# fractalclockwork/CS267_HW3

Hardware: NVIDIA B200
Metric: kmers_per_s_insert_plus_traverse (higher is better)
Workload: dtype u128

## Files before the change

### cs267_hw3_b200/csrc/capi.cu

```cuda
#include <algorithm>
#include <cmath>
#include <cstdio>
#include <cstdlib>
#include <cstring>
#include <string>
#include <vector>

#include <cub/device/device_radix_sort.cuh>

#include "../../include/kh_capi.h"
#include "kernels.cuh"
#include "ctable.cuh"

using namespace kh;

namespace {

struct DevBuf {
    void* p = nullptr;
    size_t cap = 0;
};

enum { EV_INS0, EV_INS1, EV_AS0, EV_WALK, EV_RANK, EV_AS1, EV_PACK0, EV_PACK1, EV_CLR0, EV_CLR1, EV_STAGE1, EV_BUILD0, EV_BUILD1, EV_COUNT };

// ... 672 lines not shown
template <int W>
int ct_assemble_part(kh_table* t, int part) {
    typedef typename Slot<W>::value_t V;
    auto& c = t->ct;
    const unsigned gb = (unsigned)t->sm_count * 8;
    u64* link = static_cast<u64*>(t->link.p);
    CtGathered gt = {};
    for (int r = 0; r < c.pe.world; ++r) {
        const bool me = r == c.pe.rank;
        gt.link[r] = me ? link : static_cast<const u64*>(c.g_link.p) + (u64)r * c.caps.g_seg_stride;
        gt.meta[r] = me ? static_cast<const u64*>(c.meta.p) : static_cast<const u64*>(c.g_meta.p) + (u64)r * c.caps.g_seg_stride;
        gt.pool[r] = me ? static_cast<const unsigned char*>(c.pool.p) : static_cast<const unsigned char*>(c.g_pool.p) + (u64)r * c.caps.g_pool_stride;
    }
    switch (part) {
    case 0:
        if (c.assembled) { c.sealed = false; c.assembled = false; }
        c.slow = false;
        KH_CUDA(t, cudaEventRecord(t->ev[EV_AS0], t->stream));
        if (!c.sealed) return ct_seal_publish<W>(t);
        return ct_barrier(t);
    case 1: {
        if (!c.sealed) { KH_TRY(ct_seal_build<W>(t)); KH_CUDA(t, cudaEventRecord(t->ev[EV_INS1], t->stream)); t->have_ins = true; }
        if (!c.sharded) {
            const u64 hc = c.n_starts_host;
            KH_TRY(ensure(t, t->contig_len, (hc + 3) * sizeof(u32)));
            KH_TRY(ensure(t, t->contig_pre, (hc + 3) * sizeof(u32)));
            KH_TRY(ensure(t, t->contig_off, (hc + 3) * sizeof(u64)));
            c.out_cap = t->h_ctr->n_inserted + c.n_starts_host * (u64)(t->k + 1) + 64;
            ct_set_self(t);
        }
        if (c.pe.world > 1) {
            KH_CUDA(t, cudaEventRecord(t->ev_built, t->stream));
            KH_CUDA(t, cudaStreamWaitEvent(t->copy_stream, t->ev_built, 0));
            ct_gather_kernel<<<gb, 256, 0, t->copy_stream>>>(c.pe, c.caps, link, static_cast<const u64*>(c.meta.p), static_cast<const unsigned char*>(c.pool.p),
                                                             static_cast<const u32*>(c.pool_off.p), c.g.chunks_per_rank, t->d_ctr, 0);
            KH_CUDA(t, cudaEventRecord(t->ev_gathered, t->copy_stream));
            ++t->n_launches;
        }
        ct_init_assemble_kernel<<<1, 1, 0, t->stream>>>(t->d_ctr);
        KH_CUDA(t, cudaMemsetAsync(c.out_cursor.p, 0, kMaxRanks * sizeof(u32), t->stream));
        ct_stub_kernel<W><<<std::max(1u, std::min(gb, (c.caps.hcap + 255u) / 256u)), 256, 0, t->stream>>>(
            static_cast<const V*>(t->starts.p), t->d_ctr, c.caps.hcap, link, static_cast<u64*>(c.meta.p), static_cast<V*>(c.ext_key.p));
        ct_resolve_kernel<W><<<gb, 256, 0, t->stream>>>(static_cast<const V*>(t->table), static_cast<const u32*>(c.chunk_base.p),
                                                        static_cast<const u32*>(c.seg_base.p), link, static_cast<const V*>(c.ext_key.p),
                                                        c.g, c.pe, c.caps, static_cast<u32*>(c.out_cursor.p), static_cast<u32*>(c.req_seg.p), t->d_ctr);
        if (c.pe.world > 1) { ct_publish_inbox_kernel<<<1, 32, 0, t->stream>>>(c.pe, c.caps, static_cast<const u32*>(c.out_cursor.p)); ++t->n_launches; }
        t->n_launches += 3;
        KH_CUDA(t, cudaGetLastError());
        return ct_barrier(t);
    }
    case 2:
        if (c.pe.world > 1) {
            ct_answer_kernel<W><<<gb, 256, 0, t->stream>>>(static_cast<const V*>(t->table), static_cast<const u32*>(c.chunk_base.p),
                                                           static_cast<const u32*>(c.seg_base.p), static_cast<const CtReq<W>*>(c.inbox.p),
                                                           static_cast<const u32*>(c.inbox_cnt.p), c.g, c.pe, c.caps);
            KH_CUDA(t, cudaGetLastError());
            ++t->n_launches;
        }
        return ct_barrier(t);
    case 3:
        if (c.pe.world > 1) {
            ct_apply_kernel<<<gb, 256, 0, t->stream>>>(link, static_cast<const u32*>(c.answers.p), static_cast<const u32*>(c.req_seg.p),
                                                       static_cast<const u32*>(c.out_cursor.p), c.caps, c.pe.world, c.pe.rank);
            ct_gather_kernel<<<gb, 256, 0, t->stream>>>(c.pe, c.caps, link, static_cast<const u64*>(c.meta.p), static_cast<const unsigned char*>(c.pool.p),
                                                        static_cast<const u32*>(c.pool_off.p), c.g.chunks_per_rank, t->d_ctr, 1);
            KH_CUDA(t, cudaStreamWaitEvent(t->stream, t->ev_gathered, 0));
            KH_CUDA(t, cudaGetLastError());
            t->n_launches += 2;
        }
        KH_CUDA(t, cudaEventRecord(t->ev[EV_WALK], t->stream));
        return ct_barrier(t);
    case 4:
        ct_walk_len_kernel<<<gb, 256, 0, t->stream>>>(gt, link, c.caps, t->k, kCtWalkMaxSteps, static_cast<u32*>(t->contig_len.p), t->d_ctr);
        KH_CUDA(t, cudaGetLastError());
        ++t->n_launches;
        return ct_barrier(t, -2);
    case 5: {
        KH_TRY(device_scan(t, static_cast<u32*>(t->contig_len.p), (u64)c.caps.hcap + 1, static_cast<u64*>(t->contig_off.p), &t->d_ctr->contig_bytes));
        KH_CUDA(t, cudaEventRecord(t->ev[EV_RANK], t->stream));
        ct_walk_emit_kernel<W><<<gb, 256, 0, t->stream>>>(gt, link, static_cast<const V*>(t->starts.p), c.caps, t->k, static_cast<const u32*>(t->contig_len.p),
                                                          static_cast<const u64*>(t->contig_off.p), c.out_cap, static_cast<char*>(t->out.p), t->d_ctr);
        KH_CUDA(t, cudaGetLastError());
        ++t->n_launches;
        KH_CUDA(t, cudaEventRecord(t->ev[EV_AS1], t->stream));
        t->have_as = true;
        return KH_OK;
    }
    case 6: {
        KH_TRY(read_counters(t));
        c.slow = (c.pe.world > 1 ? t->h_ctr->use_jump : t->h_ctr->need_jump) != 0;
        if (!c.slow) return KH_OK;
        c.assembled = true;
        ct_rank_round_kernel<<<gb, 256, 0, t->stream>>>(c.pe, link, c.caps, t->d_ctr, t->d_ctr->flags, 0);
        KH_CUDA(t, cudaGetLastError());
        ++t->n_launches;
        return ct_barrier(t, 0);
    }
    case 6 + kCtMaxRounds: {
        if (!c.slow) return KH_OK;
        ct_reset_nodes_kernel<<<1, 1, 0, t->stream>>>(t->d_ctr);
        ct_lengths_kernel<<<gb, 256, 0, t->stream>>>(c.pe, link, c.caps, t->k, static_cast<u32*>(t->contig_len.p),
                                                     static_cast<u32*>(t->contig_pre.p), t->d_ctr);
        ct_claim_kernel<<<gb, 256, 0, t->stream>>>(c.pe, link, c.caps, static_cast<const u32*>(t->contig_len.p), t->d_ctr);
        KH_CUDA(t, cudaGetLastError());
        t->n_launches += 3;
        KH_TRY(device_scan(t, static_cast<u32*>(t->contig_len.p), (u64)c.caps.hcap + 1, static_cast<u64*>(t->contig_off.p), &t->d_ctr->contig_bytes));
        KH_CUDA(t, cudaEventRecord(t->ev[EV_RANK], t->stream));
        return ct_barrier(t);
    }
    case 7 + kCtMaxRounds:
        if (!c.slow) return KH_OK;
        ct_emit_kernel<<<gb, 256, 0, t->stream>>>(c.pe, link, static_cast<const u64*>(c.meta.p), static_cast<const unsigned char*>(c.pool.p),
                                                  c.caps, t->d_ctr, t->k);
        ct_emit_heads_kernel<W><<<gb, 256, 0, t->stream>>>(static_cast<const V*>(t->starts.p), c.caps, t->k, static_cast<const u32*>(t->contig_len.p),
                                                          static_cast<const u64*>(t->contig_off.p), t->d_ctr, c.out_cap, static_cast<char*>(t->out.p));
        KH_CUDA(t, cudaGetLastError());
        t->n_launches += 2;
        KH_CUDA(t, cudaEventRecord(t->ev[EV_AS1], t->stream));
        t->have_as = true;
        return ct_barrier(t);
    default: {
        if (part < 7 || part >= 6 + kCtMaxRounds) return fail(t, KH_ERR_ARG, "unknown assemble part");
        if (!c.slow) return KH_OK;
        const int r = part - 6;
        ct_rank_round_kernel<<<gb, 256, 0, t->stream>>>(c.pe, link, c.caps, t->d_ctr, t->d_ctr->flags, r);
        KH_CUDA(t, cudaGetLastError());
        ++t->n_launches;
        return ct_barrier(t, r);
    }
    }
}

int ct_finish(kh_table* t, u32* bits_out) {
    auto& c = t->ct;
    KH_TRY(read_counters(t));
    const Counters& h = *t->h_ctr;
    const u64 n_starts = std::min<u64>(h.n_starts_dev, c.caps.hcap);
    t->n_starts = n_starts;
    t->stats.n_contigs = n_starts;
    t->stats.n_nodes = h.n_nodes;
    t->stats.contig_bytes = h.contig_bytes;
    t->stats.n_segments = (h.next_seg > c.caps.hcap ? h.next_seg - c.caps.hcap : 0) + n_starts;
    u32 rounds = 0;
    for (int i = 0; i < kCtMaxRounds; ++i) rounds += h.flags[i] ? 1u : 0u;
    t->stats.rank_rounds = rounds + 1;
    t->last_contig_bytes = h.contig_bytes;
    t->last_n_contigs = n_starts;
    u32 e = h.errors;
    if (e == 0 && h.contig_bytes > c.out_cap) e = kErrConverge;
    if (bits_out) *bits_out = e;
    if (e & kErrInternal) {
        char msg[512];
        snprintf(msg, sizeof msg, "rank %d/%d internal error, site bits 0x%x (1 barrier wait, 2 start list, 4 segment ids, 8 link inbox, "
                 "16 unresolved head stub, 32 output buffer): starts %llu/%u, segments %u/%u, contig bytes %llu/%llu, epoch %u",
                 c.pe.rank, c.pe.world, h.err_where, (unsigned long long)h.n_starts_dev, c.caps.hcap, h.next_seg, c.caps.seg_cap,
                 (unsigned long long)h.contig_bytes, (unsigned long long)c.out_cap, c.epoch);
        t->err = msg;
        fprintf(stderr, "libkh_b200: %s\n", msg);
    }
    if (h.errors) { clear_error_bits(t); KH_CUDA(t, cudaMemsetAsync(&t->d_ctr->err_where, 0, sizeof(u32), t->stream)); }
    return KH_OK;
}

template <int W>
int ct_insert_plain(kh_table* t, const unsigned char* recs, u64 n, bool record_start) {
    auto& c = t->ct;
    if (record_start) KH_CUDA(t, cudaEventRecord(t->ev[EV_INS0], t->stream));
    KH_TRY(ct_stage<W>(t, recs, n));
    KH_TRY(read_counters(t));
    c.n_starts_host = std::min<u64>(t->h_ctr->n_starts_dev, 0xFFFFFF00ull);
    t->n_starts = c.n_starts_host;
    KH_CUDA(t, cudaEventRecord(t->ev[EV_INS1], t->stream));
    t->have_ins = true;
    const u32 e = t->h_ctr->errors;
    if (e) { clear_error_bits(t); return status_from_errors(t, e); }
    return KH_OK;
}

template <int W>
int ct_seal_plain(kh_table* t) {
    auto& c = t->ct;
    if (c.sealed) return KH_OK;
    KH_TRY(ct_seal_publish<W>(t));
    KH_TRY(ct_seal_build<W>(t));
    KH_CUDA(t, cudaEventRecord(t->ev[EV_INS1], t->stream));
    KH_TRY(read_counters(t));
    const u32 e = t->h_ctr->errors;
    if (e) { clear_error_bits(t); return status_from_errors(t, e); }
    return KH_OK;
}

template <int W>
int ct_assemble_plain(kh_table* t) {
    auto& c = t->ct;
    if (c.assembled) { c.sealed = false; c.assembled = false; }
    KH_TRY(ct_seal_plain<W>(t));
    KH_TRY(ensure(t, t->out, t->h_ctr->n_inserted + c.n_starts_host * (u64)(t->k + 1) + 64));
    for (int part = 0; part < kCtParts; ++part) KH_TRY(ct_assemble_part<W>(t, part));
    u32 bits = 0;
    KH_TRY(ct_finish(t, &bits));
    if (bits) return status_from_errors(t, bits);
    return KH_OK;
}

}

extern "C" {

int kh_abi_version(void) { return 2; }

int kh_device_count(void) {
    int n = 0;
    if (cudaGetDeviceCount(&n) != cudaSuccess) { cudaGetLastError(); return 0; }
    return n;
}

const char* kh_status_string(int s) {
    switch (s) {
    case KH_OK: return "ok";
    case KH_ERR_ARG: return "bad argument";
    case KH_ERR_CUDA: return "CUDA failure or no CUDA device";
    case KH_ERR_NOT_FOUND: return "Error: k-mer not found in Distributed HashMap.";
    case KH_ERR_TABLE_FULL: return "hash table full";
    case KH_ERR_CYCLE: return "chain never terminates (cycle)";
    case KH_ERR_BAD_INPUT: return "malformed input";
    case KH_ERR_CONVERGE: return "chains are not linear (shared end node)";
    case KH_ERR_NOMEM: return "out of memory";
    default: return "unknown status";
    }
}

uint64_t kh_packed_bytes(int k) { return (uint64_t)((k + 3) / 4); }
uint64_t kh_pair_bytes(int k) { return (uint64_t)((k + 3) / 4 + 2); }

int kh_create(int k, uint64_t n_expected, double load_factor, int device, kh_table** out) {
    if (!out) return KH_ERR_ARG;
    *out = nullptr;
    if (k < 2 || k > 61 || !(load_factor > 0.0) || load_factor > 1.0) return KH_ERR_ARG;
    int ndev = 0;
    if (cudaGetDeviceCount(&ndev) != cudaSuccess || ndev == 0) { cudaGetLastError(); return KH_ERR_CUDA; }
    if (device < 0 || device >= ndev) return KH_ERR_ARG;
    kh_table* t = new kh_table();
    auto bail = [&](int rc) { kh_destroy(t); return rc; };
    t->k = k; t->device = device; t->lf = load_factor; t->n_expected = n_expected;
    t->pl = (k + 3) / 4; t->pb = t->pl + 2;
    t->ct_env = env_int("KH_CT", 1);
    const bool use_ct = ct_supported(k) && (t->ct_env == 2 || (t->ct_env != 0 && n_expected >= (1ull << 20) && 2 * k + 6 > 64));
    t->W = use_ct ? ct_slot_words(k) : ((2 * k + 6 <= 64) ? 1 : 2);
    t->slot_bytes = t->W == 1 ? 8 : 16;
    t->per_bucket = 32 / t->slot_bytes;
    if (cudaSetDevice(device) != cudaSuccess) return bail(KH_ERR_CUDA);
    cudaDeviceProp prop;
    if (cudaGetDeviceProperties(&prop, device) != cudaSuccess) return bail(KH_ERR_CUDA);
    if (prop.major < 9) { fprintf(stderr, "libkh_b200: device %d is sm_%d%d; this library is built for sm_100a only\n", device, prop.major, prop.minor); return bail(KH_ERR_CUDA); }
    t->sm_count = prop.multiProcessorCount;
    const int gran = env_int("KH_L2_FETCH_BYTES", 32);
    if (gran > 0) { cudaDeviceSetLimit(cudaLimitMaxL2FetchGranularity, (size_t)gran); cudaGetLastError(); }

    const long double slots = (long double)std::max<uint64_t>(n_expected, 1) / (long double)load_factor;
    t->nbuckets = std::max<u64>(16, (u64)(slots / t->per_bucket) + 1);
    t->nbuckets = (t->nbuckets + 15) / 16 * 16;
    t->table_bytes = use_ct ? 0 : (size_t)t->nbuckets * 32;
    int rc = KH_OK;
    auto ck = [&](cudaError_t e) { if (e != cudaSuccess && rc == KH_OK) { rc = e == cudaErrorMemoryAllocation ? KH_ERR_NOMEM : KH_ERR_CUDA; t->err = cudaGetErrorString(e); } };
    ck(cudaStreamCreateWithFlags(&t->own_stream, cudaStreamNonBlocking));
    ck(cudaStreamCreateWithFlags(&t->copy_stream, cudaStreamNonBlocking));
    t->stream = t->own_stream;
    if (!use_ct) ck(cudaMalloc(&t->table, t->table_bytes));
    ck(cudaMalloc((void**)&t->d_ctr, sizeof(Counters)));
    ck(cudaHostAlloc((void**)&t->h_ctr, sizeof(Counters), cudaHostAllocDefault));
    for (auto& e : t->ev) ck(cudaEventCreate(&e));
    for (auto& e : t->ev_copied) ck(cudaEventCreateWithFlags(&e, cudaEventDisableTiming));
    for (auto& e : t->ev_consumed) ck(cudaEventCreateWithFlags(&e, cudaEventDisableTiming));
    ck(cudaEventCreateWithFlags(&t->ev_built, cudaEventDisableTiming));
    ck(cudaEventCreateWithFlags(&t->ev_gathered, cudaEventDisableTiming));
    if (rc != KH_OK) { fprintf(stderr, "libkh_b200: kh_create: %s\n", t->err.c_str()); return bail(rc); }
    if (!use_ct) ck(cudaMemsetAsync(t->table, 0, t->table_bytes, t->stream));
    ck(cudaMemsetAsync(t->d_ctr, 0, sizeof(Counters), t->stream));
    ck(cudaStreamSynchronize(t->stream));
    if (rc != KH_OK) return bail(rc);
    memset(t->h_ctr, 0, sizeof(Counters));
    int v = env_int("KH_SPLIT_BUCKETS", 0);
    if (v > 0 && set_option(t, "split_buckets", v) != KH_OK) fprintf(stderr, "libkh_b200: ignoring KH_SPLIT_BUCKETS=%d\n", v);
    t->partition_mode = env_int("KH_PARTITION", -1);
    t->build_mode = env_int("KH_BUILD", t->W == 1 ? 1 : 0);
    t->debug_cap_pct = std::max(1, env_int("KH_DEBUG_CAP_PCT", 100));
    v = env_int("KH_SEG_CHARS", 0);
    if (v > 0 && set_option(t, "seg_chars", v) != KH_OK) fprintf(stderr, "libkh_b200: ignoring KH_SEG_CHARS=%d\n", v);
    if (use_ct) {
        rc = t->W == 1 ? ct_setup<1>(t, 0, 1, n_expected, n_expected, n_expected, false)
                       : ct_setup<2>(t, 0, 1, n_expected, n_expected, n_expected, false);
        if (rc != KH_OK) { fprintf(stderr, "libkh_b200: kh_create: %s\n", t->err.c_str()); return bail(rc); }
    }
    t->err.clear();
    *out = t;
    return KH_OK;
}

int kh_destroy(kh_table* t) {
    if (!t) return KH_OK;
    cudaSetDevice(t->device);
    if (t->own_stream) cudaStreamSynchronize(t->own_stream);
    DevBuf* bufs[] = {&t->starts, &t->mask, &t->tile_counts, &t->tile_offs, &t->scan_blocks, &t->link, &t->seglen,
                      &t->tmp, &t->part_cursor, &t->grouped, &t->fine, &t->chunk_cursor, &t->overflow, &t->contig_len, &t->contig_pre, &t->contig_off, &t->out, &t->stage[0], &t->stage[1],
                      &t->text_stage, &t->scratch_a, &t->scratch_b, &t->scratch_c, &t->sort_keys[0], &t->sort_keys[1], &t->sort_vals[0], &t->sort_vals[1], &t->sort_tmp};
    for (DevBuf* b : bufs) if (b->p) cudaFree(b->p);
    for (auto& row : t->ct.ipc_opened) for (void* q : row) if (q) cudaIpcCloseMemHandle(q);
// ... 596 lines not shown
```

### cs267_hw3_b200/csrc/ctable.cuh

```cuda
#pragma once
#include "kernels.cuh"

namespace kh {

#ifndef KH_CT_BUCKETS2
#define KH_CT_BUCKETS2 2176
#endif
#ifndef KH_CT_THREADS
#define KH_CT_THREADS 512
#endif
#ifndef KH_CT_MINBLOCKS
#define KH_CT_MINBLOCKS 2
#endif
#ifndef KH_CT_JUMPS
#define KH_CT_JUMPS 3
#endif
template <int W> struct CtBuild {
    static constexpr u32 kMaxBuckets = (W == 1) ? 1536u : (u32)KH_CT_BUCKETS2;
    static constexpr u32 kMaxSlots = kMaxBuckets * (u32)Slot<W>::kPerBucket;
    static constexpr u32 kOffSucc = kMaxBuckets * 32u;
    static constexpr u32 kOffPd = kOffSucc + kMaxSlots * 2u;
    static constexpr u32 kOffOff = kOffPd + kMaxSlots * 4u;
    static constexpr u32 kOffCode = kOffOff + kMaxSlots * 2u;
    static constexpr u32 kSmem = kOffCode + kMaxSlots;
};
constexpr int kCtBuildThreads = KH_CT_THREADS;
template <int W>
__host__ __device__ __forceinline__ u64 ct_fine_index(u32 chunk, u32 at, u32 nchunks) {
    constexpr u32 G = 128u / (u32)sizeof(typename Slot<W>::value_t);
    return ((u64)(at / G) * nchunks + chunk) * G + (at % G);
}
constexpr u32 kSuccExt = 0x8000u, kSuccTail = 0xFFFFu, kSuccDead = 0xFFFDu, kPredNone = 0xFFFFu;
constexpr u32 kCodeBackF = 8u, kCodeMulti = 16u;

template <int W> struct CtReq;
template <> struct alignas(16) CtReq<1> { u64 key; u32 src; u32 chunk; };
template <> struct alignas(16) CtReq<2> { u128 key; u32 src; u32 chunk; u64 pad; };

struct CtPeers {
    int world, rank;
    void* xin_vals[kMaxRanks];
    u32* xin_chunk[kMaxRanks];
    u32* xin_cnt[kMaxRanks];
    void* extra_vals[kMaxRanks];
    u32* extra_chunk[kMaxRanks];
    u32* extra_cnt[kMaxRanks];
    u64* link[kMaxRanks];
    u64* meta[kMaxRanks];
    void* inbox[kMaxRanks];
    u32* inbox_cnt[kMaxRanks];
    u32* answers[kMaxRanks];
    u64* g_link[kMaxRanks];
    u64* g_meta[kMaxRanks];
    unsigned char* g_pool[kMaxRanks];
    u32* g_hdr[kMaxRanks];
    u32* contig_pre[kMaxRanks];
    u64* contig_off[kMaxRanks];
    char* out[kMaxRanks];
    u64 out_cap[kMaxRanks];
    u32* flags[kMaxRanks];
};

struct CtCaps {
    u32 xin_cap, extra_cap, inbox_cap, seg_cap, hcap;
    u64 nbuckets_alloc, pool_cap;
    u64 g_seg_stride, g_pool_stride;
};

__device__ __forceinline__ void ct_internal(Counters* ctr, u32 site) {
    atomicOr(&ctr->errors, kErrInternal);
    atomicOr(&ctr->err_where, site);
}

__global__ void ct_barrier_kernel(const CtPeers pe, u32 epoch, Counters* ctr, int round) {
    const int r = (int)threadIdx.x;
    if (round >= 0 && ctr->rank_done) return;
    const u32 bit = round >= 0 ? (ctr->flags[round] ? 1u : 0u) : (round == -2 ? (ctr->need_jump ? 1u : 0u) : 0u);
    u32 peer_bit = 0;
    if (r < pe.world) {
        __threadfence_system();
        u32* dst = pe.flags[r] + 2 * pe.rank + (epoch & 1u);
        asm volatile("st.release.sys.global.u32 [%0], %1;" ::"l"(dst), "r"((epoch << 1) | bit) : "memory");
        const u32* src = pe.flags[pe.rank] + 2 * r + (epoch & 1u);
        unsigned long long t0, t1;
        asm volatile("mov.u64 %0, %%globaltimer;" : "=l"(t0));
        for (;;) {
            u32 seen;
            asm volatile("ld.acquire.sys.global.u32 %0, [%1];" : "=r"(seen) : "l"(src) : "memory");
            if ((int)((seen >> 1) - epoch) >= 0) { peer_bit = ((seen >> 1) == epoch) ? (seen & 1u) : (round >= 0 ? 0u : 1u); break; }
            asm volatile("mov.u64 %0, %%globaltimer;" : "=l"(t1));
            if (t1 - t0 > 4000000000ull) { ct_internal(ctr, kSiteBarrier); peer_bit = 1; break; }
            __nanosleep(200);
        }
        __threadfence_system();
    }
    if (round >= 0) {
        const u32 any = __ballot_sync(kFullMask, peer_bit != 0);
        if (r == 0 && any == 0) ctr->rank_done = 1;
    } else if (round == -2) {
        const u32 any = __ballot_sync(kFullMask, peer_bit != 0);
        if (r == 0) ctr->use_jump = any ? 1u : 0u;
    }
}

template <int W> __device__ __forceinline__ typename Slot<W>::value_t ct_record_from_words(const u32 (&w)[W == 1 ? 3 : 5], u32 sh, int k, int pl, bool& ok);
template <> __device__ __forceinline__ u64 ct_record_from_words<1>(const u32 (&w)[3], u32 sh, int k, int pl, bool& ok) {
    const u32 b0 = __funnelshift_r(w[0], w[1], sh), b1 = __funnelshift_r(w[1], w[2], sh);
    const u64 be = ((u64)__byte_perm(b0, 0, 0x0123) << 32) | (u64)__byte_perm(b1, 0, 0x0123);
    const u64 key = be >> (64 - 2 * k);
    const u32 ext = (u32)((((u64)b1 << 32) | b0) >> (8 * pl));
    const u32 b = ext_code((unsigned char)ext), f = ext_code((unsigned char)(ext >> 8));
    ok = (b != kExtBad) && (f != kExtBad);
    return (key << 6) | ((u64)(b & 7u) << 3) | (u64)((f + 1u) & 7u);
}
template <> __device__ __forceinline__ u128 ct_record_from_words<2>(const u32 (&w)[5], u32 sh, int k, int pl, bool& ok) {
    const u32 b0 = __funnelshift_r(w[0], w[1], sh), b1 = __funnelshift_r(w[1], w[2], sh);
    const u32 b2 = __funnelshift_r(w[2], w[3], sh), b3 = __funnelshift_r(w[3], w[4], sh);
    const u64 hi = ((u64)__byte_perm(b0, 0, 0x0123) << 32) | (u64)__byte_perm(b1, 0, 0x0123);
    const u64 lo = ((u64)__byte_perm(b2, 0, 0x0123) << 32) | (u64)__byte_perm(b3, 0, 0x0123);
    u128 v = Slot<2>::shr_any(u128{lo, hi}, 122 - 2 * k);
    const int wq = pl >> 2;
    const u32 e0 = wq == 1 ? b1 : (wq == 2 ? b2 : b3), e1 = wq == 1 ? b2 : (wq == 2 ? b3 : 0u);
    const u32 ext = __funnelshift_r(e0, e1, 8u * (pl & 3));
    const u32 b = ext_code((unsigned char)ext), f = ext_code((unsigned char)(ext >> 8));
    ok = (b != kExtBad) && (f != kExtBad);
    v.lo = (v.lo & ~63ull) | ((u64)(b & 7u) << 3) | (u64)((f + 1u) & 7u);
    return v;
}

constexpr int kStgThreads = 256;
constexpr int kStgPer = 4;
constexpr int kStgTile = kStgThreads * kStgPer;

template <int W>
__global__ void __launch_bounds__(kStgThreads, 5)
ct_stage_kernel(const unsigned char* __restrict__ recs, u64 n, const CtGeom g, const CtPeers pe, const CtCaps caps,
                u32* __restrict__ chunk_cursor, typename Slot<W>::value_t* __restrict__ fine, u32* __restrict__ xout_cursor,
                u32* __restrict__ start_mask, u32* __restrict__ tile_starts, Counters* ctr) {
    typedef Slot<W> S;
    typedef typename S::value_t V;
    constexpr u32 kMaxSlots = CtBuild<W>::kMaxSlots;
    extern __shared__ __align__(16) unsigned char s_raw[];
    V* s_sorted = reinterpret_cast<V*>(s_raw);
    u32* s_schunk = reinterpret_cast<u32*>(s_raw + (size_t)kStgTile * sizeof(V));
    __shared__ u32 s_cnt[kMaxRanks], s_off[kMaxRanks + 1], s_gbase[kMaxRanks];
    __shared__ u32 s_starts[kStgTile / kInsTile], s_err;
    const int k = g.k, pl = (k + 3) >> 2, pb = pl + 2;
    const u64 rec0 = (u64)blockIdx.x * kStgTile;
    const u32 cnt = (u32)min((u64)kStgTile, n - rec0);
    const bool multi = g.world > 1;
    if (threadIdx.x < kMaxRanks) s_cnt[threadIdx.x] = 0;
    if (threadIdx.x < kStgTile / kInsTile) s_starts[threadIdx.x] = 0;
    if (threadIdx.x == 0) s_err = 0;
    constexpr int kWords = W == 1 ? 3 : 5;
    u32 raw[kStgPer][kWords];
    u32 shift[kStgPer];
#pragma unroll
    for (int r = 0; r < kStgPer; ++r) {
        const u32 j = threadIdx.x + r * kStgThreads;
        const u64 addr = reinterpret_cast<u64>(recs) + (rec0 + j) * (u64)pb;
        shift[r] = ((u32)addr & 3u) * 8u;
        const u32* wp = reinterpret_cast<const u32*>(addr & ~3ull);
        const u64 end = reinterpret_cast<u64>(recs) + n * (u64)pb;
#pragma unroll
        for (int q = 0; q < kWords; ++q)
            raw[r][q] = (j < cnt && reinterpret_cast<u64>(wp + q) < end) ? __ldg(wp + q) : 0u;
    }
    __syncthreads();
    V v[kStgPer];
    u32 dst[kStgPer];
    u32 at[kStgPer];
    u32 own[kStgPer];
    u32 err = 0;
#pragma unroll
    for (int r = 0; r < kStgPer; ++r) {
        const u32 j = threadIdx.x + r * kStgThreads;
        bool ok = true, live = j < cnt;
        dst[r] = 0xFFFFFFFFu; own[r] = 0xFFFFFFFFu; at[r] = 0;
        v[r] = ct_record_from_words<W>(raw[r], shift[r], k, pl, ok);
        if (!live) v[r] = S::zero();
        if (live && !ok) { err |= kErrBadInput; live = false; }
        if (live) {
            u32 owner, chunk;
            ct_place(ct_min_hash<W>(v[r], g.m, g.win), g, owner, chunk);
            dst[r] = chunk;
            if (!multi || owner == (u32)g.rank) at[r] = atomicAdd(&chunk_cursor[chunk], 1u);
// ... 255 lines not shown
        const bool m = (((q[i] ^ key) << kIdxBits) >> (kIdxBits + 6)) == 0ull;
        res = e ? kFindMiss : (m ? (int)(q[i] >> (64 - kIdxBits)) - 1 : res);
    }
    return res;
}
template <> __device__ __forceinline__ int ct_find_step<2>(unsigned saddr, u128 key) {
    u64 q[4];
    ct_lds_bucket<2>(saddr, q);
    int res = kFindNext;
#pragma unroll
    for (int i = 1; i >= 0; --i) {
        const bool e = ((u32)q[2 * i] & 7u) == 0u;
        const bool m = (((q[2 * i + 1] ^ key.hi) << kIdxBits) | ((q[2 * i] ^ key.lo) >> 6)) == 0ull;
        res = e ? kFindMiss : (m ? (int)(q[2 * i + 1] >> (64 - kIdxBits)) - 1 : res);
    }
    return res;
}

template <int W>
__global__ void __launch_bounds__(kCtBuildThreads, KH_CT_MINBLOCKS)
ct_build_kernel(const typename Slot<W>::value_t* __restrict__ fine, const u32* __restrict__ chunk_cursor,
                const u32* __restrict__ chunk_base, const u32* __restrict__ pool_off,
                typename Slot<W>::value_t* __restrict__ table, u32* __restrict__ seg_base,
                u64* __restrict__ link, u64* __restrict__ meta, typename Slot<W>::value_t* __restrict__ ext_key,
                unsigned char* __restrict__ pool, const CtGeom g, const CtCaps caps, Counters* ctr) {
    typedef Slot<W> S;
    typedef CtSlot<W> CS;
    typedef typename S::value_t V;
    typedef CtBuild<W> B;
    extern __shared__ __align__(128) unsigned char s_bld[];
    unsigned char* const s_raw = s_bld;
    V* s_tab = reinterpret_cast<V*>(s_raw);
    unsigned short* s_succ = reinterpret_cast<unsigned short*>(s_raw + B::kOffSucc);
    unsigned char* s_pool = s_raw + B::kOffSucc;
    u32* s_pd = reinterpret_cast<u32*>(s_raw + B::kOffPd);
    unsigned short* s_off = reinterpret_cast<unsigned short*>(s_raw + B::kOffOff);
    unsigned char* s_code = s_raw + B::kOffCode;
    __shared__ u32 s_inserted, s_dups, s_nheads, s_seg0, s_chars, s_err;
    const u32 c = blockIdx.x;
    const u32 b0 = chunk_base[c], nb = chunk_base[c + 1] - b0;
    const u32 cnt = min(chunk_cursor[c], B::kMaxSlots);
    if (nb == 0) {
        if (threadIdx.x == 0) seg_base[c] = 0;
        return;
    }
    const unsigned s_base = (unsigned)__cvta_generic_to_shared(s_tab);
    const int k = g.k;
    constexpr int kBatch = 4;
    V v[kBatch];
#pragma unroll
    for (int r = 0; r < kBatch; ++r) {
        const u32 i = threadIdx.x + r * kCtBuildThreads;
        v[r] = i < cnt ? fine[ct_fine_index<W>(c, i, g.chunks_per_rank)] : S::zero();
    }
    if (threadIdx.x == 0) { s_inserted = 0; s_dups = 0; s_nheads = 0; s_chars = 0; s_err = 0; }
    {
        uint4* s4 = reinterpret_cast<uint4*>(s_raw);
        for (u32 i = threadIdx.x; i < nb * 2u; i += kCtBuildThreads) s4[i] = make_uint4(0, 0, 0, 0);
        for (u32 i = threadIdx.x; i < cnt; i += kCtBuildThreads) s_pd[i] = (kPredNone << 16) | 1u;
    }
    __syncthreads();
    u32 inserted = 0, dups = 0, err = 0;
    for (u32 base = 0; base < cnt; base += kCtBuildThreads * kBatch) {
        V nxt[kBatch];
#pragma unroll
        for (int r = 0; r < kBatch; ++r) {
            const u32 i = base + kCtBuildThreads * kBatch + threadIdx.x + r * kCtBuildThreads;
            nxt[r] = i < cnt ? fine[ct_fine_index<W>(c, i, g.chunks_per_rank)] : S::zero();
        }
#pragma unroll
        for (int r = 0; r < kBatch; ++r) {
            const u32 node = base + threadIdx.x + r * kCtBuildThreads;
            if (node >= cnt) continue;
            const int slot = ct_smem_insert<W>(s_tab, s_base, nb, CS::with_idx(v[r], node + 1u));
            inserted += (slot >= 0);
            dups += (slot == -1);
            if (slot == -2) err |= kErrTableFull;
            s_succ[node] = (unsigned short)(slot >= 0 ? (u32)slot : kSuccDead);
        }
#pragma unroll
        for (int r = 0; r < kBatch; ++r) v[r] = nxt[r];
    }
    inserted = __reduce_add_sync(kFullMask, inserted);
    dups = __reduce_add_sync(kFullMask, dups);
    err = __reduce_or_sync(kFullMask, err);
    if (lane_id() == 0) {
        if (inserted) atomicAdd(&s_inserted, inserted);
        if (dups) atomicAdd(&s_dups, dups);
        if (err) atomicOr(&s_err, err);
    }
    __syncthreads();
#pragma unroll 1
    for (u32 base = threadIdx.x; base < cnt; base += 2 * kCtBuildThreads) {
        u32 slot[2], b[2], code[2];
        V key[2];
        int res[2];
#pragma unroll
        for (int q = 0; q < 2; ++q) {
            const u32 node = base + q * kCtBuildThreads;
            slot[q] = node < cnt ? (u32)s_succ[node] : kSuccDead;
        }
#pragma unroll
        for (int q = 0; q < 2; ++q) {
            const V cur = slot[q] != kSuccDead ? s_tab[slot[q]] : S::zero();
            const u32 f = slot[q] != kSuccDead ? S::fwd(cur) : kExtF;
            code[q] = f | ((slot[q] != kSuccDead && S::back(cur) == kExtF) ? kCodeBackF : 0u);
            key[q] = S::next_key(CS::strip(cur), k);
            b[q] = ct_bucket_in_chunk(CS::hash32(key[q]), nb);
        }
#pragma unroll
        for (int q = 0; q < 2; ++q) res[q] = (code[q] & 7u) != kExtF ? ct_find_step<W>(s_base + b[q] * 32u, key[q]) : kFindMiss;
#pragma unroll
        for (int q = 0; q < 2; ++q) {
            for (u32 tries = 1; res[q] == kFindNext && tries < nb; ++tries) {
                b[q] = (b[q] + 1 == nb) ? 0u : b[q] + 1;
                res[q] = ct_find_step<W>(s_base + b[q] * 32u, key[q]);
            }
        }
#pragma unroll
        for (int q = 0; q < 2; ++q) {
            const u32 node = base + q * kCtBuildThreads;
            if (node >= cnt) continue;
            s_code[node] = (unsigned char)code[q];
            u32 sc = slot[q] == kSuccDead ? kSuccDead : kSuccTail;
            if ((code[q] & 7u) != kExtF) {
                if (res[q] < 0) {
                    sc = kSuccExt | slot[q];
                } else {
                    sc = (u32)res[q];
                    s_pd[res[q]] = (node << 16) | 1u;
                }
            }
            s_succ[node] = (unsigned short)sc;
        }
    }
    __syncthreads();
#pragma unroll 1
    for (u32 node = threadIdx.x; node < cnt; node += kCtBuildThreads) {
        const u32 s = s_succ[node];
        if (s < kSuccExt && (s_pd[s] >> 16) != node) s_code[s] |= (unsigned char)kCodeMulti;
    }
    __syncthreads();
    for (u32 base = 0; base < cnt; base += kCtBuildThreads) {
        const u32 node = base + threadIdx.x;
        bool head = false, dead = true;
        if (node < cnt) {
            dead = s_succ[node] == kSuccDead;
            head = !dead && ((s_pd[node] >> 16) == kPredNone || (s_code[node] & (kCodeBackF | kCodeMulti)));
        }
        const u32 bal = __ballot_sync(kFullMask, head);
        u32 first = 0;
        if (lane_id() == 0 && bal) first = atomicAdd(&s_nheads, (u32)__popc(bal));
        first = __shfl_sync(kFullMask, first, 0);
        if (head) s_pd[node] = (node << 16) | (first + __popc(bal & ((1u << lane_id()) - 1u)));
        else if (dead && node < cnt) s_pd[node] = node << 16;
    }
    __syncthreads();
    const u32 nheads = s_nheads;
    if (threadIdx.x == 0) {
        u32 seg0 = nheads ? atomicAdd(&ctr->next_seg, nheads) : 0u;
        if (seg0 + nheads > caps.seg_cap) { ct_internal(ctr, kSiteSegCap); seg0 = caps.seg_cap; }
        s_seg0 = seg0;
        seg_base[c] = seg0;
    }
    u32 active = 0;
#pragma unroll 1
    for (u32 i = 0, node = threadIdx.x; node < cnt; ++i, node += kCtBuildThreads) {
        const u32 pd = s_pd[node];
        active |= ((pd >> 16) != node) ? (1u << i) : 0u;
    }
    for (int round = 0; round < (14 + KH_CT_JUMPS - 1) / KH_CT_JUMPS; ++round) {
#pragma unroll 1
        for (int rep = 0; rep < KH_CT_JUMPS; ++rep) {
#pragma unroll 1
            for (u32 m = active; m; m &= m - 1u) {
                const u32 i = (u32)__ffs((int)m) - 1u, node = threadIdx.x + i * kCtBuildThreads;
                const u32 pd = s_pd[node], a = pd >> 16;
                const u32 pa = s_pd[a], a2 = pa >> 16;
                if (a2 == a) { active &= ~(1u << i); continue; }
                s_pd[node] = (a2 << 16) | ((pd + pa) & 0xFFFFu);
            }
        }
        if (!__syncthreads_or(active != 0u)) break;
    }
    __syncthreads();
    const u32 seg0 = s_seg0;
    const u32 my_bits = (u32)g.rank << kRankShift;
    const u64 pool0 = pool_off[c];
    if (seg0 < caps.seg_cap) {
    #pragma unroll 1
    for (u32 node = threadIdx.x; node < cnt; node += kCtBuildThreads) {
            const u32 s = s_succ[node];
            if (s == kSuccDead) continue;
            const u32 pd = s_pd[node], a = pd >> 16;
            const bool root = a == node;
            const u32 pa = root ? pd : s_pd[a];
            if ((pa >> 16) != a) continue;
            const u32 f = s_code[node] & 7u;
            bool last = f == kExtF || s >= kSuccExt;
            u32 next_hi = f == kExtF ? kLinkTail : kLinkPending;
            if (!last) {
                const u32 ps = s_pd[s];
                if ((ps >> 16) == s) { last = true; next_hi = my_bits | (seg0 + (ps & 0xFFFFu)); }
            }
            if (!last) continue;
            const u32 n = (root ? 0u : (pd & 0xFFFFu)) + (f != kExtF ? 1u : 0u);
            const u32 off = atomicAdd(&s_chars, n);
            s_off[a] = (unsigned short)off;
            const u32 gseg = seg0 + (pa & 0xFFFFu);
            link[gseg] = ((u64)next_hi << 32) | (next_hi == kLinkTail ? 0u : n);
            meta[gseg] = ((pool0 + off) << 24) | n;
            if (next_hi == kLinkPending) ext_key[gseg] = S::next_key(CS::strip(s_tab[s & 0x7FFFu]), k);
        }
    }
    __syncthreads();
#pragma unroll 1
    for (u32 node = threadIdx.x; node < cnt; node += kCtBuildThreads) {
        const u32 code = s_code[node];
        if ((code & 7u) == kExtF) continue;
        const u32 pd = s_pd[node], a = pd >> 16;
        const bool root = a == node;
        if (!root && (s_pd[a] >> 16) != a) continue;
        s_pool[(u32)s_off[a] + (root ? 0u : (pd & 0xFFFFu))] = ext_char(code & 7u);
    }
    {
        const u32 nslots = nb * S::kPerBucket;
        for (u32 i = threadIdx.x; i < nslots; i += kCtBuildThreads) {
            const V cur = s_tab[i];
            if (S::empty(cur)) continue;
            const u32 node = CS::idx(cur) - 1u, pd = s_pd[node];
            s_tab[i] = CS::with_idx(cur, (pd >> 16) == node ? (pd & 0xFFFFu) + 1u : 0u);
        }
    }
    asm volatile("fence.proxy.async.shared::cta;" ::: "memory");
    __syncthreads();
    {
        const u32 tab_bytes = nb * 32u, pool_bytes = (s_chars + 15u) & ~15u;
        constexpr u32 kPiece = 8192u;
        const u32 tab_pieces = (tab_bytes + kPiece - 1u) / kPiece, pool_pieces = (pool_bytes + kPiece - 1u) / kPiece;
        if (lane_id() == 0) {
            unsigned char* g_tab = reinterpret_cast<unsigned char*>(table + (u64)b0 * S::kPerBucket);
            bool any = false;
            for (u32 pc = threadIdx.x >> 5; pc < tab_pieces + pool_pieces; pc += kCtBuildThreads / 32) {
                const bool is_tab = pc < tab_pieces;
                const u32 o = (is_tab ? pc : pc - tab_pieces) * kPiece;
                const u32 bytes = min(kPiece, (is_tab ? tab_bytes : pool_bytes) - o);
                const unsigned src = (unsigned)__cvta_generic_to_shared(is_tab ? s_raw + o : s_pool + o);
                unsigned char* dst = is_tab ? g_tab + o : pool + pool0 + o;
                asm volatile("cp.async.bulk.global.shared::cta.bulk_group [%0], [%1], %2;" ::"l"(dst), "r"(src), "r"(bytes) : "memory");
                any = true;
            }
            if (any) {
                asm volatile("cp.async.bulk.commit_group;" ::: "memory");
                asm volatile("cp.async.bulk.wait_group.read 0;" ::: "memory");
            }
        }
    }
    if (threadIdx.x == 0) {
        if (s_inserted) atomicAdd(&ctr->n_inserted, (u64)s_inserted);
        if (s_dups) atomicAdd(&ctr->n_duplicates, (u64)s_dups);
        if (s_err) atomicOr(&ctr->errors, s_err);
    }
}

template <int W>
__device__ __forceinline__ bool ct_lookup_chunk(const typename Slot<W>::value_t* __restrict__ table, const u32* __restrict__ chunk_base,
                                                u32 chunk, typename Slot<W>::value_t key, typename Slot<W>::value_t& found) {
    typedef Slot<W> S;
    typedef typename S::value_t V;
    const u32 b0 = chunk_base[chunk], nb = chunk_base[chunk + 1] - b0;
    if (nb == 0) return false;
    u32 b = ct_bucket_in_chunk(CtSlot<W>::hash32(key), nb);
    for (u32 tries = 0; tries < nb; ++tries) {
        u64 q[4];
        load256_nc(table + (u64)(b0 + b) * S::kPerBucket, q);
        bool hole = false, hit = false;
#pragma unroll
        for (int i = 0; i < S::kPerBucket; ++i) {
            const V cur = S::from_bucket(q, i);
            const bool e = S::empty(cur);
            if (!hole && !hit && !e && CtSlot<W>::same_key(cur, key)) { found = cur; hit = true; }
            hole = hole || e;
        }
        if (hit) return true;
        if (hole) return false;
        b = (b + 1 == nb) ? 0u : b + 1;
    }
    return false;
}

template <int W>
__global__ void __launch_bounds__(256)
ct_find_kernel(const typename Slot<W>::value_t* __restrict__ table, const u32* __restrict__ chunk_base, const CtGeom g,
               const unsigned char* __restrict__ pkmers, u64 n, unsigned char* __restrict__ pairs_out,
               unsigned char* __restrict__ found_out) {
    typedef Slot<W> S;
    const u64 i = (u64)blockIdx.x * blockDim.x + threadIdx.x;
    if (i >= n) return;
    const int k = g.k, pl = (k + 3) >> 2, pb = pl + 2;
    unsigned char key[16];
    for (int j = 0; j < pl; ++j) key[j] = pkmers[i * pl + j];
    const typename S::value_t kb = S::from_packed(key, k, pl);
    u32 owner, chunk;
    ct_place(ct_min_hash<W>(kb, g.m, g.win), g, owner, chunk);
    typename S::value_t hit;
    const bool ok = ct_lookup_chunk<W>(table, chunk_base, chunk, kb, hit);
    unsigned char rec[18];
    for (int j = 0; j < pb; ++j) rec[j] = 0;
    if (ok) S::to_record(CtSlot<W>::strip(hit), k, pl, rec);
    for (int j = 0; j < pb; ++j) pairs_out[i * pb + j] = rec[j];
    found_out[i] = ok ? 1 : 0;
}

template <int W>
__global__ void __launch_bounds__(256)
ct_stub_kernel(const typename Slot<W>::value_t* __restrict__ starts, const Counters* __restrict__ ctr, u32 hcap,
               u64* __restrict__ link, u64* __restrict__ meta, typename Slot<W>::value_t* __restrict__ ext_key) {
    typedef Slot<W> S;
    const u32 n_starts = (u32)min(ctr->n_starts_dev, (u64)hcap);
    for (u32 c = blockIdx.x * blockDim.x + threadIdx.x; c < hcap; c += gridDim.x * blockDim.x) {
        if (c < n_starts) {
            link[c] = (u64)kLinkPending << 32;
            meta[c] = 0;
            ext_key[c] = S::key_only(starts[c]);
        } else {
            link[c] = (u64)kLinkUnused << 32;
        }
    }
}

template <int W>
__device__ __forceinline__ u32 ct_resolve_one(const typename Slot<W>::value_t* __restrict__ table, const u32* __restrict__ chunk_base,
                                              const u32* __restrict__ seg_base, u32 chunk, typename Slot<W>::value_t key, u32 my_bits) {
    typename Slot<W>::value_t hit;
    if (!ct_lookup_chunk<W>(table, chunk_base, chunk, key, hit)) return kLinkMissing;
    const u32 idx = CtSlot<W>::idx(hit);
    if (idx == 0) return kLinkConverge;
    return my_bits | (seg_base[chunk] + idx - 1u);
}

constexpr int kResPerThread = 4;
constexpr int kResTile = 256 * kResPerThread;
template <int W>
__global__ void __launch_bounds__(256)
ct_resolve_kernel(const typename Slot<W>::value_t* __restrict__ table, const u32* __restrict__ chunk_base,
                  const u32* __restrict__ seg_base, u64* __restrict__ link, const typename Slot<W>::value_t* __restrict__ ext_key,
                  const CtGeom g, const CtPeers pe, const CtCaps caps, u32* __restrict__ out_cursor, u32* __restrict__ req_seg, Counters* ctr) {
    typedef Slot<W> S;
    typedef typename S::value_t V;
    __shared__ u32 s_cnt[kMaxRanks], s_base[kMaxRanks];
    const u32 nseg = min(ctr->next_seg, caps.seg_cap);
    const u32 my_bits = (u32)g.rank << kRankShift;
    const u32 ntiles = (nseg + kResTile - 1) / kResTile;
    for (u32 tile = blockIdx.x; tile < ntiles; tile += gridDim.x) {
        if (threadIdx.x < kMaxRanks) s_cnt[threadIdx.x] = 0;
        __syncthreads();
        CtReq<W> e[kResPerThread];
        u32 dest[kResPerThread], rk[kResPerThread];
#pragma unroll
        for (int r = 0; r < kResPerThread; ++r) {
            const u32 s = tile * kResTile + r * 256 + threadIdx.x;
            u32 d = 0xFFFFFFFFu;
            if (s < nseg && (u32)(link[s] >> 32) == kLinkPending) {
                const V key = ext_key[s];
                u32 owner, chunk;
                ct_place(ct_min_hash<W>(key, g.m, g.win), g, owner, chunk);
                if (owner == (u32)g.rank) {
                    reinterpret_cast<u32*>(link + s)[1] = ct_resolve_one<W>(table, chunk_base, seg_base, chunk, key, my_bits);
                } else {
                    d = owner;
                    e[r].key = key; e[r].src = my_bits | s; e[r].chunk = chunk;
                }
            }
            dest[r] = d;
            const unsigned same = __match_any_sync(kFullMask, d);
            const int leader = __ffs(same) - 1;
// ... 358 lines not shown
```

### cs267_hw3_b200/csrc/slot.cuh

```cuda
#pragma once
#include <cstdint>
#include <cuda_runtime.h>

namespace kh {

typedef unsigned long long u64;
typedef unsigned int u32;

constexpr u32 kExtF = 4;
constexpr u32 kExtBad = 7;

struct alignas(16) u128 {
    u64 lo, hi;
};

constexpr u64 ext_lut_entry(u64 lut, int idx, u64 code) { return (lut & ~(7ull << (3 * idx))) | (code << (3 * idx)); }
constexpr u64 kExtLut = ext_lut_entry(ext_lut_entry(ext_lut_entry(ext_lut_entry(ext_lut_entry(
                            0x7FFFFFFFFFFFFFFFull, 1, 0), 3, 1), 6, 4), 7, 2), 20, 3);
__host__ __device__ __forceinline__ u32 ext_code(unsigned char c) {
    const u32 i = c & 31u;
    const bool letter = (c & 0xE0u) == 0x40u && i <= 20u;
    return letter ? ((u32)(kExtLut >> (3u * i)) & 7u) : kExtBad;
}
#ifdef __CUDACC__
// ... 228 lines not shown
    static __device__ __forceinline__ value_t cas_shared(value_t* addr, value_t expect, value_t val) {
        u128 old;
        const unsigned saddr = (unsigned)__cvta_generic_to_shared(addr);
        asm volatile("{\n\t.reg .b128 c, v, o;\n\tmov.b128 c, {%2, %3};\n\tmov.b128 v, {%4, %5};\n\t"
                     "atom.shared.cas.b128 o, [%6], c, v;\n\tmov.b128 {%0, %1}, o;\n\t}"
                     : "=l"(old.lo), "=l"(old.hi)
                     : "l"(expect.lo), "l"(expect.hi), "l"(val.lo), "l"(val.hi), "r"(saddr) : "memory");
        return old;
    }
    static __device__ __forceinline__ value_t load_shared(const value_t* addr) {
        const volatile u64* p = reinterpret_cast<const volatile u64*>(addr);
        return u128{p[0], p[1]};
    }
};


__host__ __device__ __forceinline__ u64 bucket_of(u64 h, u64 nbuckets) {
#ifdef __CUDA_ARCH__
    return __umul64hi(h, nbuckets);
#else
    return (u64)(((unsigned __int128)h * nbuckets) >> 64);
#endif
}

template <int W>
__host__ __device__ __forceinline__ u64 place_bucket(typename Slot<W>::value_t v, u64 nbuckets) {
    return bucket_of(Slot<W>::hash(v), nbuckets);
}

constexpr u32 kIdxBits = 14;
constexpr u32 kMinMul = 0x9E3779B1u;
constexpr u32 kMinAdd = 0x7F4A7C15u;

__host__ __device__ __forceinline__ int ct_minimizer_len(int k) { return k >= 31 ? 15 : (k >= 23 ? 13 : (k >= 17 ? k - 6 : k)); }
__host__ __device__ __forceinline__ int ct_window(int k) { const int w = k - ct_minimizer_len(k) + 1; return w > 32 ? 32 : w; }
__host__ __device__ __forceinline__ bool ct_supported(int k) { return k >= 17 && k <= 54; }
__host__ __device__ __forceinline__ int ct_slot_words(int k) { return (2 * k + 6 + (int)kIdxBits <= 64) ? 1 : 2; }

__host__ __device__ __forceinline__ u32 ct_funnel_r(u32 lo, u32 hi, u32 s) {
#ifdef __CUDA_ARCH__
    return __funnelshift_r(lo, hi, s);
#else
    return s ? ((lo >> s) | (hi << (32 - s))) : lo;
#endif
}
__host__ __device__ __forceinline__ u32 ct_mulhi32(u32 a, u32 b) {
#ifdef __CUDA_ARCH__
    return __umulhi(a, b);
#else
    return (u32)(((u64)a * b) >> 32);
#endif
}
__host__ __device__ __forceinline__ u32 ct_min_hash_words(u32 a, u32 b, u32 c, u32 d, int m, int win) {
    const u32 mul = kMinMul << (32 - 2 * m);
    u32 best = 0xFFFFFFFFu;
    int rem = win;
    for (int it = 0; it < 2; ++it) {
        if (rem >= 16) {
#pragma unroll
            for (int j = 0; j < 16; ++j) {
                const u32 h = ct_funnel_r(a, b, 2u * j) * mul + kMinAdd;
                best = h < best ? h : best;
            }
        } else {
#pragma unroll
            for (int j = 0; j < 16; ++j) {
                u32 h = ct_funnel_r(a, b, 2u * j) * mul + kMinAdd;
                h = (j < rem) ? h : 0xFFFFFFFFu;
                best = h < best ? h : best;
            }
        }
        if (rem <= 16) break;
        rem -= 16; a = b; b = c; c = d; d = 0;
    }
    return best;
}
template <int W> __host__ __device__ __forceinline__ u32 ct_min_hash(typename Slot<W>::value_t v, int m, int win);
template <> __host__ __device__ __forceinline__ u32 ct_min_hash<1>(u64 v, int m, int win) {
    const u64 key = v >> 6;
    return ct_min_hash_words((u32)key, (u32)(key >> 32), 0u, 0u, m, win);
}
template <> __host__ __device__ __forceinline__ u32 ct_min_hash<2>(u128 v, int m, int win) {
    const u64 lo = (v.lo >> 6) | (v.hi << 58), hi = v.hi >> 6;
    return ct_min_hash_words((u32)lo, (u32)(lo >> 32), (u32)hi, (u32)(hi >> 32), m, win);
}

__host__ __device__ __forceinline__ u32 ct_fmix32_hi(u32 h) {
    h ^= h >> 15; h *= 0x85EBCA6Bu;
    h ^= h >> 13; h *= 0xC2B2AE35u;
    return h;
}
template <int W> struct CtSlot;
template <> struct CtSlot<1> {
    typedef u64 V;
    static __host__ __device__ __forceinline__ V strip(V v) { return v & (~0ull >> kIdxBits); }
    static __host__ __device__ __forceinline__ u32 idx(V v) { return (u32)(v >> (64 - kIdxBits)); }
    static __host__ __device__ __forceinline__ V with_idx(V v, u32 i) { return strip(v) | ((u64)i << (64 - kIdxBits)); }
    static __host__ __device__ __forceinline__ bool same_key(V a, V b) { return (((a ^ b) << kIdxBits) >> (kIdxBits + 6)) == 0ull; }
    static __host__ __device__ __forceinline__ u32 hash32(V v) {
        const u32 x0 = (u32)v & ~63u, x1 = (u32)(v >> 32) & (0xFFFFFFFFu >> kIdxBits);
        return ct_fmix32_hi((x0 * 0x9E3779B1u) ^ x1);
    }
};
template <> struct CtSlot<2> {
    typedef u128 V;
    static __host__ __device__ __forceinline__ V strip(V v) { return u128{v.lo, v.hi & (~0ull >> kIdxBits)}; }
    static __host__ __device__ __forceinline__ u32 idx(V v) { return (u32)(v.hi >> (64 - kIdxBits)); }
    static __host__ __device__ __forceinline__ V with_idx(V v, u32 i) { return u128{v.lo, (v.hi & (~0ull >> kIdxBits)) | ((u64)i << (64 - kIdxBits))}; }
    static __host__ __device__ __forceinline__ bool same_key(V a, V b) { return (((a.hi ^ b.hi) << kIdxBits) | ((a.lo ^ b.lo) >> 6)) == 0ull; }
    static __host__ __device__ __forceinline__ u32 hash32(V v) {
        const u32 x0 = (u32)v.lo & ~63u, x1 = (u32)(v.lo >> 32), x2 = (u32)v.hi, x3 = (u32)(v.hi >> 32) & (0xFFFFFFFFu >> kIdxBits);
        u32 h = x0 * 0x9E3779B1u;
        h = (h ^ x1) * 0x85EBCA77u;
        h = (h ^ x2) * 0xC2B2AE3Du;
        return ct_fmix32_hi(h ^ x3);
    }
};
__host__ __device__ __forceinline__ u32 ct_bucket_in_chunk(u32 h32, u32 nb) { return ct_mulhi32(h32, nb); }

struct CtGeom {
    int k, m, win;
    int world, rank;
    u32 chunks_per_rank;
    u32 max_buckets;
    u32 lf_inv_q16;
};
__host__ __device__ __forceinline__ void ct_place(u32 minhash, const CtGeom& g, u32& owner, u32& chunk) {
    const u32 u = ct_fmix32_hi(minhash ^ (minhash >> 16));
    owner = ct_mulhi32(u, (u32)g.world);
    chunk = ct_mulhi32(u, (u32)g.world * g.chunks_per_rank) - owner * g.chunks_per_rank;
}

constexpr int kMaxRanks = 8;
constexpr u32 kRankShift = 28;
constexpr u32 kLocalMask = (1u << kRankShift) - 1u;
constexpr u32 kLinkFinalBit = 0x80000000u;
constexpr u32 kLinkDistMask = 0x7FFFFFFFu;
constexpr u32 kLinkMissing = 0xFFFFFFFBu;
constexpr u32 kLinkConverge = 0xFFFFFFFAu;
constexpr u32 kLinkLoop = kLinkConverge;
constexpr u32 kLinkCtFirstMarker = kLinkConverge;

enum : u32 {
    kErrNotFound = 1u, kErrTableFull = 2u, kErrCycle = 4u, kErrBadInput = 8u,
    kErrConverge = 16u, kErrInternal = 32u
};

constexpr u32 kLinkTail = 0xFFFFFFFFu;
constexpr u32 kLinkUnused = 0xFFFFFFFEu;
constexpr u32 kLinkClaimed = 0xFFFFFFFDu;
constexpr u32 kLinkPending = 0xFFFFFFFCu;
constexpr u32 kLinkFirstMarker = kLinkPending;

enum : u32 { kSiteBarrier = 1u, kSiteStarts = 2u, kSiteSegCap = 4u, kSiteInbox = 8u, kSiteStubOpen = 16u, kSiteOutCap = 32u };

struct Counters {
    u32 next_walker;
    u32 next_seg;
    u32 errors;
    u32 rank_rounds;
    u64 n_inserted;
    u64 n_duplicates;
    u64 scan_total;
    u64 n_nodes;
    u64 contig_bytes;
    u32 n_outbox;
    u32 flags[40];
    u32 rank_done;
    u32 err_where;
    u64 n_starts_dev;
    u32 need_jump;
    u32 use_jump;
};

}
```

Measured before the change: 12.67 billion.

## Replace pointer-jumping segment ranking with per-head serial walks in CT build

The build kernel used to rank nodes into segments with repeated shared-memory pointer jumping over all nodes, taking several barrier-synchronised rounds. It now gives each segment head to one lane, which walks the successor chain serially and writes each node's head and distance. A warp prefix-scan then reserves pool offsets for the segments. This drops the log-depth jumping rounds and the extra root-finding pass, but work per lane now scales with segment length, so long segments cause imbalance and warp divergence. A walk-length guard with a new internal error site is added.

```diff
diff --git a/cs267_hw3_b200/csrc/capi.cu b/cs267_hw3_b200/csrc/capi.cu
--- a/cs267_hw3_b200/csrc/capi.cu
+++ b/cs267_hw3_b200/csrc/capi.cu
@@ -848,7 +848,7 @@
     if (e & kErrInternal) {
         char msg[512];
         snprintf(msg, sizeof msg, "rank %d/%d internal error, site bits 0x%x (1 barrier wait, 2 start list, 4 segment ids, 8 link inbox, "
-                 "16 unresolved head stub, 32 output buffer): starts %llu/%u, segments %u/%u, contig bytes %llu/%llu, epoch %u",
+                 "16 unresolved head stub, 32 output buffer, 64 segment walk in the build): starts %llu/%u, segments %u/%u, contig bytes %llu/%llu, epoch %u",
                  c.pe.rank, c.pe.world, h.err_where, (unsigned long long)h.n_starts_dev, c.caps.hcap, h.next_seg, c.caps.seg_cap,
                  (unsigned long long)h.contig_bytes, (unsigned long long)c.out_cap, c.epoch);
         t->err = msg;
diff --git a/cs267_hw3_b200/csrc/ctable.cuh b/cs267_hw3_b200/csrc/ctable.cuh
--- a/cs267_hw3_b200/csrc/ctable.cuh
+++ b/cs267_hw3_b200/csrc/ctable.cuh
@@ -11,9 +11,6 @@
 #endif
 #ifndef KH_CT_MINBLOCKS
 #define KH_CT_MINBLOCKS 2
-#endif
-#ifndef KH_CT_JUMPS
-#define KH_CT_JUMPS 3
 #endif
 template <int W> struct CtBuild {
     static constexpr u32 kMaxBuckets = (W == 1) ? 1536u : (u32)KH_CT_BUCKETS2;
@@ -31,7 +28,8 @@
     return ((u64)(at / G) * nchunks + chunk) * G + (at % G);
 }
 constexpr u32 kSuccExt = 0x8000u, kSuccTail = 0xFFFFu, kSuccDead = 0xFFFDu, kPredNone = 0xFFFFu;
-constexpr u32 kCodeBackF = 8u, kCodeMulti = 16u;
+constexpr u32 kPdUnreached = (kPredNone << 16) | 0xFFFFu;
+constexpr u32 kCodeBackF = 8u, kCodeMulti = 16u, kCodeHead = 32u;
 
 template <int W> struct CtReq;
 template <> struct alignas(16) CtReq<1> { u64 key; u32 src; u32 chunk; };
@@ -593,8 +591,14 @@
         u32 first = 0;
         if (lane_id() == 0 && bal) first = atomicAdd(&s_nheads, (u32)__popc(bal));
         first = __shfl_sync(kFullMask, first, 0);
-        if (head) s_pd[node] = (node << 16) | (first + __popc(bal & ((1u << lane_id()) - 1u)));
-        else if (dead && node < cnt) s_pd[node] = node << 16;
+        if (head) {
+            const u32 j = first + __popc(bal & ((1u << lane_id()) - 1u));
+            s_pd[node] = (node << 16) | j;
+            s_off[j] = (unsigned short)node;
+            s_code[node] |= (unsigned char)kCodeHead;
+        } else if (node < cnt) {
+            s_pd[node] = dead ? node << 16 : kPdUnreached;
+        }
     }
     __syncthreads();
     const u32 nheads = s_nheads;
@@ -604,54 +608,48 @@
         s_seg0 = seg0;
         seg_base[c] = seg0;
     }
-    u32 active = 0;
-#pragma unroll 1
-    for (u32 i = 0, node = threadIdx.x; node < cnt; ++i, node += kCtBuildThreads) {
-        const u32 pd = s_pd[node];
-        active |= ((pd >> 16) != node) ? (1u << i) : 0u;
-    }
-    for (int round = 0; round < (14 + KH_CT_JUMPS - 1) / KH_CT_JUMPS; ++round) {
-#pragma unroll 1
-        for (int rep = 0; rep < KH_CT_JUMPS; ++rep) {
-#pragma unroll 1
-            for (u32 m = active; m; m &= m - 1u) {
-                const u32 i = (u32)__ffs((int)m) - 1u, node = threadIdx.x + i * kCtBuildThreads;
-                const u32 pd = s_pd[node], a = pd >> 16;
-                const u32 pa = s_pd[a], a2 = pa >> 16;
-                if (a2 == a) { active &= ~(1u << i); continue; }
-                s_pd[node] = (a2 << 16) | ((pd + pa) & 0xFFFFu);
-            }
-        }
-        if (!__syncthreads_or(active != 0u)) break;
-    }
     __syncthreads();
     const u32 seg0 = s_seg0;
     const u32 my_bits = (u32)g.rank << kRankShift;
     const u64 pool0 = pool_off[c];
-    if (seg0 < caps.seg_cap) {
-    #pragma unroll 1
-    for (u32 node = threadIdx.x; node < cnt; node += kCtBuildThreads) {
-            const u32 s = s_succ[node];
-            if (s == kSuccDead) continue;
-            const u32 pd = s_pd[node], a = pd >> 16;
-            const bool root = a == node;
-            const u32 pa = root ? pd : s_pd[a];
-            if ((pa >> 16) != a) continue;
-            const u32 f = s_code[node] & 7u;
-            bool last = f == kExtF || s >= kSuccExt;
-            u32 next_hi = f == kExtF ? kLinkTail : kLinkPending;
-            if (!last) {
-                const u32 ps = s_pd[s];
-                if ((ps >> 16) == s) { last = true; next_hi = my_bits | (seg0 + (ps & 0xFFFFu)); }
-            }
-            if (!last) continue;
-            const u32 n = (root ? 0u : (pd & 0xFFFFu)) + (f != kExtF ? 1u : 0u);
-            const u32 off = atomicAdd(&s_chars, n);
-            s_off[a] = (unsigned short)off;
-            const u32 gseg = seg0 + (pa & 0xFFFFu);
-            link[gseg] = ((u64)next_hi << 32) | (next_hi == kLinkTail ? 0u : n);
-            meta[gseg] = ((pool0 + off) << 24) | n;
-            if (next_hi == kLinkPending) ext_key[gseg] = S::next_key(CS::strip(s_tab[s & 0x7FFFu]), k);
+#pragma unroll 1
+    for (u32 base = threadIdx.x & ~31u; base < nheads; base += kCtBuildThreads) {
+        const u32 j = base + lane_id();
+        u32 n = 0, next_hi = 0, s = 0;
+        if (j < nheads) {
+            const u32 h = s_off[j];
+            u32 code = s_code[h], d = 0;
+            s = s_succ[h];
+            while ((code & 7u) != kExtF && s < kSuccExt) {
+                const u32 cs = s_code[s];
+                if (cs & kCodeHead) break;
+                if (++d >= cnt) { ct_internal(ctr, kSiteSegWalk); break; }
+                s_pd[s] = (h << 16) | d;
+                code = cs;
+                s = s_succ[s];
+            }
+            const u32 f = code & 7u;
+            n = d + (f != kExtF ? 1u : 0u);
+            next_hi = f == kExtF ? kLinkTail : (s >= kSuccExt ? kLinkPending : my_bits | (seg0 + (s_pd[s] & 0xFFFFu)));
+        }
+        u32 incl = n;
+#pragma unroll
+        for (u32 o = 1; o < 32; o <<= 1) {
+            const u32 t = __shfl_up_sync(kFullMask, incl, o);
+            if (lane_id() >= o) incl += t;
+        }
+        u32 wbase = 0;
+        if (lane_id() == 31 && incl) wbase = atomicAdd(&s_chars, incl);
+        wbase = __shfl_sync(kFullMask, wbase, 31);
+        if (j < nheads) {
+            const u32 off = wbase + incl - n;
+            s_off[j] = (unsigned short)off;
+            if (seg0 < caps.seg_cap) {
+                const u32 gseg = seg0 + j;
+                link[gseg] = ((u64)next_hi << 32) | (next_hi == kLinkTail ? 0u : n);
+                meta[gseg] = ((pool0 + off) << 24) | n;
+                if (next_hi == kLinkPending) ext_key[gseg] = S::next_key(CS::strip(s_tab[s & 0x7FFFu]), k);
+            }
         }
     }
     __syncthreads();
@@ -660,9 +658,10 @@
         const u32 code = s_code[node];
         if ((code & 7u) == kExtF) continue;
         const u32 pd = s_pd[node], a = pd >> 16;
+        if (a == kPredNone) continue;
         const bool root = a == node;
-        if (!root && (s_pd[a] >> 16) != a) continue;
-        s_pool[(u32)s_off[a] + (root ? 0u : (pd & 0xFFFFu))] = ext_char(code & 7u);
+        const u32 j = (root ? pd : s_pd[a]) & 0xFFFFu;
+        s_pool[(u32)s_off[j] + (root ? 0u : (pd & 0xFFFFu))] = ext_char(code & 7u);
     }
     {
         const u32 nslots = nb * S::kPerBucket;
diff --git a/cs267_hw3_b200/csrc/slot.cuh b/cs267_hw3_b200/csrc/slot.cuh
--- a/cs267_hw3_b200/csrc/slot.cuh
+++ b/cs267_hw3_b200/csrc/slot.cuh
@@ -404,7 +404,7 @@
 constexpr u32 kLinkPending = 0xFFFFFFFCu;
 constexpr u32 kLinkFirstMarker = kLinkPending;
 
-enum : u32 { kSiteBarrier = 1u, kSiteStarts = 2u, kSiteSegCap = 4u, kSiteInbox = 8u, kSiteStubOpen = 16u, kSiteOutCap = 32u };
+enum : u32 { kSiteBarrier = 1u, kSiteStarts = 2u, kSiteSegCap = 4u, kSiteInbox = 8u, kSiteStubOpen = 16u, kSiteOutCap = 32u, kSiteSegWalk = 64u };
 
 struct Counters {
     u32 next_walker;
```

Result: faster. 13.33 billion (median of 6 runs) (+5.2%).
